# yardenas/ethz-safe-learning

Measured on AMD Instinct MI355X. Metric: planning steps/sec (CEM-MPC, N=2000 K=5 H=30), higher is better.
Workload: dtype f32

## Files before the change

### ethz_safe_learning_amd/_capi.py

```python
from __future__ import annotations

import ctypes as C
import os

CEM_ABI_VERSION = 4
CEM_MAX_ACT = 32
CEM_MAX_COST_KINDS = 4
CEM_COMM_ID_BYTES = 128
CEM_MAX_BATCH = 256
CEM_TRAIN_MAX_BATCH = 4096
CEM_INIT_COLD, CEM_INIT_EXPLICIT, CEM_INIT_SHIFT = 0, 1, 2
CEM_VARIANT_CEM, CEM_VARIANT_SAFE, CEM_VARIANT_COST = 0, 1, 2
CEM_PARTICLES_MEAN, CEM_PARTICLES_LOWER_TAIL = 0, 1
CEM_CONSTRAINT_BETA, CEM_CONSTRAINT_BUDGET = 0, 1
CEM_REFIT_UNIFORM, CEM_REFIT_SOFTMAX = 0, 1
CEM_NOISE_WHITE, CEM_NOISE_MIXED = 0, 1
CEM_FORWARD_SPLIT, CEM_FORWARD_ALL = 0, 1

_HERE = os.path.dirname(os.path.abspath(__file__))
LIB_PATH = os.environ.get('CEM_MPC_LIB') or os.path.join(_HERE, 'lib', 'libcem_mpc_gfx950.so')

EXPORTED_SYMBOLS = [
    'cem_abi_version', 'cem_status_string', 'cem_last_hip_error', 'cem_weight_blob_floats',
    'cem_packed_weight_floats', 'cem_workspace_bytes', 'cem_pack_weights_host', 'cem_plan_tiles_host', 'cem_plan_segments_host', 'cem_rollout_residency',
    'cem_planner_create', 'cem_planner_destroy', 'cem_planner_layout', 'cem_planner_set_weights', 'cem_planner_set_weights_dev',
    'cem_planner_set_normaliser', 'cem_planner_plan', 'cem_plan_begin', 'cem_plan_rollout', 'cem_plan_select',
    'cem_plan_end', 'cem_comm_unique_id', 'cem_planner_comm_init', 'cem_planner_comm_destroy', 'cem_planner_comm_ranks', 'cem_plan_exchange', 'cem_planner_graph_status', 'cem_planner_launches_per_iteration', 'cem_planner_rollout_path', 'cem_unfold_sequences', 'cem_compute_objective', 'cem_scorer_reward', 'cem_scorer_cost', 'cem_fill_noise', 'cem_philox_words', 'cem_planner_set_timing', 'cem_planner_last_timing', 'cem_planner_last_timing_detail', 'cem_planner_select_mode', 'cem_planner_inject_fault',
    'cem_batch_workspace_bytes', 'cem_batch_planner_create', 'cem_planner_plan_batch', 'cem_planner_batch_capacity',
    'cem_planner_set_warm_start', 'cem_planner_set_initial_distribution', 'cem_planner_set_init_mode', 'cem_planner_reset_carry',
    'cem_planner_get_carry', 'cem_planner_set_carry_slots', 'cem_planner_set_particle_objective', 'cem_planner_get_particle_objective',
    'cem_planner_set_constraint', 'cem_planner_get_constraint', 'cem_planner_set_cost_budget', 'cem_planner_constraint_costs',
    'cem_planner_set_refit', 'cem_planner_get_refit', 'cem_planner_refit_stats',
    'cem_planner_set_action_noise', 'cem_planner_get_action_noise', 'cem_planner_action_noise_dev',
    'cem_planner_set_elite_carry', 'cem_planner_get_elite_carry', 'cem_planner_elite_store',
    'cem_planner_set_population_schedule', 'cem_planner_get_population_schedule', 'cem_planner_iteration_plan',
    'cem_planner_set_mean_candidate', 'cem_planner_get_mean_candidate',
    'cem_trainer_workspace_bytes', 'cem_trainer_blob_floats', 'cem_trainer_create', 'cem_trainer_destroy', 'cem_trainer_set_state',
    'cem_trainer_get_state', 'cem_trainer_weights_dev', 'cem_trainer_step', 'cem_trainer_steps', 'cem_trainer_eval', 'cem_trainer_forward',
]


class CemScorer(C.Structure):
    _fields_ = [
        ('goal_mode', C.c_int32), ('goal_lo', C.c_int32), ('goal_hi', C.c_int32),
        ('lidar_max_dist', C.c_float), ('goal_size', C.c_float), ('goal_reached_dist', C.c_float), ('reward_distance', C.c_float),
        ('reward_goal', C.c_float), ('reward_clip', C.c_float),
        ('constrain_indicator', C.c_int32), ('n_cost_kinds', C.c_int32),
        ('cost_lo', C.c_int32 * CEM_MAX_COST_KINDS), ('cost_hi', C.c_int32 * CEM_MAX_COST_KINDS),
        ('cost_size', C.c_float * CEM_MAX_COST_KINDS),
    ]
# ... 74 lines not shown
    lib.cem_plan_tiles_host.argtypes = [cfgp, i32p, i32p, vp, C.c_int32]
    lib.cem_plan_segments_host.argtypes = [cfgp, i32p, i32p]
    lib.cem_rollout_residency.argtypes = [C.c_int32, C.c_int32, i32p, i32p]
    lib.cem_planner_create.argtypes = [cfgp, vp, C.c_size_t, vp, C.POINTER(vp)]
    lib.cem_planner_destroy.argtypes = [vp]
    lib.cem_planner_layout.argtypes = [vp, C.POINTER(CemLayout)]
    lib.cem_planner_set_weights.argtypes = [vp, vp, C.c_size_t]
    lib.cem_planner_set_weights_dev.argtypes = [vp, vp, C.c_size_t]
    lib.cem_planner_set_normaliser.argtypes = [vp, vp, vp]
    lib.cem_planner_plan.argtypes = [vp, vp, C.c_uint64, C.c_uint64, vp, vp, vp, vp, fp, i32p]
    lib.cem_plan_begin.argtypes = [vp, vp, C.c_uint64, C.c_uint64, vp, vp]
    lib.cem_plan_rollout.argtypes = [vp, C.c_int32]
    lib.cem_plan_select.argtypes = [vp, C.c_int32]
    lib.cem_plan_end.argtypes = [vp, vp, vp, fp, i32p]
    lib.cem_unfold_sequences.argtypes = [vp, vp, vp, C.c_int32, C.c_int32, vp, C.c_uint64, C.c_uint64, vp, vp, vp]
    lib.cem_comm_unique_id.argtypes = [vp]
    lib.cem_planner_comm_init.argtypes = [vp, vp, C.c_int32, C.c_int32]
    lib.cem_planner_comm_destroy.argtypes = [vp]
    lib.cem_plan_exchange.argtypes = [vp]
    lib.cem_planner_graph_status.argtypes = [vp, i32p]
    lib.cem_planner_comm_ranks.argtypes = [vp, i32p]
    lib.cem_planner_launches_per_iteration.argtypes = [vp, i32p]
    lib.cem_planner_rollout_path.argtypes = [vp, i32p]
    lib.cem_compute_objective.argtypes = [vp, vp, C.c_int32, C.c_int32, vp]
    lib.cem_scorer_reward.argtypes = [vp, vp, vp, C.c_int32, vp, vp]
    lib.cem_scorer_cost.argtypes = [vp, vp, C.c_int32, vp]
    lib.cem_fill_noise.argtypes = [vp, C.c_uint64, C.c_uint64, vp, vp, vp]
    lib.cem_philox_words.argtypes = [vp, C.c_uint64, C.c_uint64] + [C.c_uint32] * 6 + [vp]
    lib.cem_planner_select_mode.argtypes = [vp, i32p]
    lib.cem_planner_inject_fault.argtypes = [vp, C.c_int32]
    lib.cem_planner_set_timing.argtypes = [vp, C.c_int32]
    lib.cem_planner_last_timing.argtypes = [vp, fp, i32p, fp]
    lib.cem_planner_last_timing_detail.argtypes = [vp, fp, fp]
    lib.cem_batch_workspace_bytes.restype = C.c_size_t
    lib.cem_batch_workspace_bytes.argtypes = [cfgp, C.c_int32]
    lib.cem_batch_planner_create.argtypes = [cfgp, C.c_int32, vp, C.c_size_t, vp, C.POINTER(vp)]
    lib.cem_planner_plan_batch.argtypes = [vp, C.c_int32, vp, C.c_uint64, vp, vp, vp, vp, vp, vp, vp]
    lib.cem_planner_batch_capacity.argtypes = [vp, i32p]
    lib.cem_planner_set_warm_start.argtypes = [vp, C.POINTER(CemWarmStart)]
    lib.cem_planner_set_initial_distribution.argtypes = [vp, C.c_int32, vp, vp]
    lib.cem_planner_set_init_mode.argtypes = [vp, C.c_int32, C.c_int32]
    lib.cem_planner_reset_carry.argtypes = [vp, C.c_int32]
    lib.cem_planner_get_carry.argtypes = [vp, C.c_int32, vp, vp, i32p]
    lib.cem_planner_set_carry_slots.argtypes = [vp, C.c_int32, vp]
    lib.cem_planner_set_particle_objective.argtypes = [vp, C.c_int32, C.c_int32]
    lib.cem_planner_get_particle_objective.argtypes = [vp, i32p, i32p]
# ... 46 lines not shown
```

### ethz_safe_learning_amd/csrc/cem_capi.hip

```cpp
#include "cem_device.h"
#include "cem_rollout_lean.h"
#include "cem_score.h"
#include "cem_refit_weighted.h"
#include "cem_noise_mix.h"
#include "cem_elite_carry.h"
#include "cem_population.h"
#include "cem_train.h"
#include "cem_train_tile.h"
#include "cem_forward.h"
#include "cem_rollout_split.h"
#include "cem_rollout_wide.h"
#include "cem_pack.h"
#include "../../include/cem_mpc.h"

#include <dlfcn.h>
#include <link.h>

#include <algorithm>
#include <atomic>
#include <chrono>
#include <cmath>
#include <cstdio>
#include <cstdlib>
#include <cstring>
// ... 572 lines not shown
}

struct IterPlan {
    Dims d;
    int rc, n_tiles, n_seg, seg_len, n_pinned;
    bool sample_in_rollout, lean_rollout;
    size_t tiles_off;
};

struct cem_planner {
    cem_config_t cfg;
    Dims d;
    Layout lay;
    char *ws;
    hipStream_t stream;
    bool own_stream;
    int rc;
    int n_tiles;
    int n_seg, seg_len, n_pinned;
    bool have_weights;
    bool in_plan;
    bool sample_in_rollout;
    bool lean_rollout;
    const float *eps_act, *eps_model;
    CtrlBlock *h_ctrl;
    float *h_result;
    WarmCtl *h_warm; const WarmCtl *d_h_warm;
    uint32_t plan_seq;
    const CtrlBlock *d_h_ctrl; float *d_h_result;
    bool timing; std::vector<hipEvent_t> ev; float roll_ms, sel_ms, red_ms, samp_ms; int roll_n;
    std::vector<std::pair<int, int>> ev_kind;
    hipGraph_t graph; hipGraphExec_t gexec; bool graph_ready;
    ScorerDev sc;
    ScorerDev sc_roll;
    float alpha, beta;
    void *comm;
    int plans_since_comm;
    bool graph_failed;
    size_t sel_dyn_limit;
    int fused_resident;
    bool sel_zeroed;
    bool fuse_banned;
    bool inject_capture_fail;
    uint32_t inject_next;
    char *scratch; size_t scratch_bytes;
    std::vector<float> h_etab;
// ... 37 lines not shown

int warm_slots(const cem_planner *h) { return h->batch ? h->batch : 1; }

bool injects_mean(const cem_planner *h, int it) { return h->mean_cand && it == h->d.I - 1; }

struct IterView {
    const Dims *d; int rc, n_tiles, n_seg, seg_len, n_pinned; bool sample_in_rollout, lean_rollout;
    const TileDesc *tiles; uint32_t *seg_flags; f4 *seg_state;
};
IterView iter_view(const cem_planner *h, int it)
{
    const Layout &l = h->lay;
    if (h->pop.empty())
        return IterView{&h->d, h->rc, h->n_tiles, h->n_seg, h->seg_len, h->n_pinned, h->sample_in_rollout, h->lean_rollout,
                        (const TileDesc *)(h->ws + l.tiles), (uint32_t *)(h->ws + l.seg_flags), (f4 *)(h->ws + l.seg_state)};
    const IterPlan &ip = h->pop[std::min(std::max(it, 0), h->d.I - 1)];
    return IterView{&ip.d, ip.rc, ip.n_tiles, ip.n_seg, ip.seg_len, ip.n_pinned, ip.sample_in_rollout, ip.lean_rollout,
                    ip.tiles_off == (size_t)-1 ? (const TileDesc *)(h->ws + l.tiles) : (const TileDesc *)(h->pop_dev + ip.tiles_off),
                    h->pop_seg_flags, h->pop_seg_state};
}

bool samples_in_rollout(const cem_planner *h, int it) { return iter_view(h, it).sample_in_rollout && h->elite.n_keep == 0 && !injects_mean(h, it); }
bool runs_lean(const cem_planner *h, int it) { return iter_view(h, it).lean_rollout && h->elite.n_keep == 0 && !injects_mean(h, it); }
int32_t *elite_counts(const cem_planner *h) { return reinterpret_cast<int32_t *>(h->elite_dev); }
size_t elite_count_floats(const cem_planner *h) { return ((size_t)warm_slots(h) + 63) & ~(size_t)63; }
float *elite_store(const cem_planner *h) { return h->elite_dev + elite_count_floats(h); }

int select_mode_for(const cem_planner *h, int N, bool *cache = nullptr)
{
    const Dims &d = h->d;
    const bool can_fuse = (N + CEM_MS_KEYS - 1) / CEM_MS_KEYS <= h->fused_resident && !h->fuse_banned;
    return resolve_select_mode(h->cfg.select_mode, N, d.k, (long long)d.H * d.A, h->sel_dyn_limit, can_fuse, cache);
}
int select_mode_now(const cem_planner *h, bool *cache = nullptr) { return select_mode_for(h, h->d.N, cache); }

void drop_graph(cem_planner *h)
{
    if (h->gexec) { hipGraphExecDestroy(h->gexec); h->gexec = nullptr; }
    if (h->graph) { hipGraphDestroy(h->graph); h->graph = nullptr; }
    h->graph_ready = false;
}

int retire_graph(cem_planner *h)
{
    if (h->graph_ready) HIPCHK(hipStreamSynchronize(h->stream));
    drop_graph(h);
// ... 130 lines not shown
    if (const char *e = std::getenv("CEM_FORCE_ROLLOUT"))
        *lean_rollout = *lean_rollout && std::strcmp(e, "generic") != 0;
}

static int planner_create(const cem_config_t *cfg, int32_t mb, void *workspace, size_t workspace_bytes, void *hip_stream, cem_planner_t **out)
{
    int st = mb ? validate_batch(cfg, mb) : validate(cfg); if (st) return st;
    if (!workspace || !out) return CEM_ERR_INVALID_ARG;
    warn_if_two_hip_runtimes();
    cem_planner *h = new (std::nothrow) cem_planner();
    if (!h) return CEM_ERR_INVALID_ARG;
    h->cfg = *cfg; h->d = make_dims(cfg);
    h->batch = mb; h->n_states = warm_slots(h);
    const size_t nb = (size_t)warm_slots(h);
    h->lay = make_layout(cfg, h->d, max_tiles_of(h->d), mb);
    if (workspace_bytes < h->lay.total || ((uintptr_t)workspace & 255)) { delete h; return CEM_ERR_WORKSPACE; }
    h->ws = (char *)workspace; h->stream = (hipStream_t)hip_stream; h->own_stream = false;
    if (!h->stream) {
        if (hipStreamCreateWithFlags(&h->stream, hipStreamNonBlocking) != hipSuccess) { g_last_hip = (int)hipGetLastError(); delete h; return CEM_ERR_HIP; }
        h->own_stream = true;
    }
    { const Plan pl = make_plan(cfg, h->d, mb); h->rc = pl.rc; h->n_seg = pl.n_seg; h->seg_len = pl.seg_len; h->n_pinned = pl.n_pinned;
      place_sampler(h, h->d, pl, &h->sample_in_rollout, &h->lean_rollout); }
    h->have_weights = false; h->in_plan = false; h->eps_act = h->eps_model = nullptr;
    h->timing = false; h->roll_ms = h->sel_ms = h->red_ms = h->samp_ms = 0.f; h->roll_n = 0;
    h->graph = nullptr; h->gexec = nullptr; h->graph_ready = false; h->tail_m = 0;
    h->cost_m = 0; h->budget_dev = nullptr; h->cstat_obj = nullptr; h->cstat_obj_n = 0; h->last_cstat = nullptr; h->last_cstat_n = h->last_cstat_problems = 0;
    h->refit_kind = CEM_REFIT_UNIFORM; h->refit_tau = 0.f; h->refit_beta = 0.f; h->refit_dev = nullptr; h->refit_ran = false;
    h->noise_kind = CEM_NOISE_WHITE; h->noise_dev = nullptr; h->noise_eps = nullptr; h->noise_floats = 0;
    h->elite = cem_elite_carry_t{}; h->elite.shift = 1; h->elite_dev = nullptr; h->elite_cap = 0; h->elite_clear = false;
    h->pop_dev = nullptr; h->pop_seg_flags = nullptr; h->pop_seg_state = nullptr; h->pop_n_ready = 0; h->mean_cand = 0;
    h->h_budget.assign(nb, std::numeric_limits<float>::infinity());
    h->comm = nullptr; h->plans_since_comm = 0; h->graph_failed = false;
    h->h_ctrl = nullptr; h->h_result = nullptr; h->h_warm = nullptr; h->d_h_warm = nullptr; h->pack_desc = nullptr; h->n_pack_desc = 0;
    h->warm = cem_warm_start_t{}; h->warm.shift = 1; h->warm_staged = 0; h->warm_save_skipped = false;
    h->slot_mode.assign(nb, CEM_INIT_COLD); h->carry_valid.assign(nb, 0); h->have_expl.assign(nb, 0); h->carry_at.assign(nb, -1);
    h->slot_of.resize(nb); for (size_t b = 0; b < nb; ++b) h->slot_of[b] = (int32_t)b;
    h->h_expl.assign(nb * 2 * h->d.H * h->d.A, 0.f);
    h->scratch = nullptr; h->scratch_bytes = 0; h->sel_zeroed = false; h->plan_seq = 0; h->fuse_banned = false; h->inject_next = 0; h->inject_capture_fail = false;
    auto fail = [&](int status) { g_last_hip = (int)hipGetLastError(); release_handle(h); return status; };
    const size_t result_bytes = mb ? nb * CEM_RESULT_WORDS * 4 : 64 * 4;
    if (hipHostMalloc((void **)&h->h_ctrl, nb * sizeof(CtrlBlock), hipHostMallocMapped | hipHostMallocCoherent) != hipSuccess ||
        hipHostMalloc((void **)&h->h_result, result_bytes, hipHostMallocMapped | hipHostMallocCoherent) != hipSuccess ||
        hipHostMalloc((void **)&h->h_warm, sizeof(WarmCtl) + nb * sizeof(WarmProb), hipHostMallocMapped | hipHostMallocCoherent) != hipSuccess) return fail(CEM_ERR_HIP);
    {
        const std::vector<PackDesc> table = build_pack_table(h->d);
// ... 428 lines not shown
    if (!samples_in_rollout(h, it)) {
        const int total = d.N * d.H * ((d.A + 3) / 4);
        TimedLaunch timed(h, 3);
        hipLaunchKernelGGL(cem_sample_kernel, dim3(std::min((total + 255) / 256, 2048), nb), dim3(256), 0, h->stream, rp);
        HIPCHK(hipGetLastError());
        rp.musig = nullptr;
        if (h->elite.n_keep && (it > 0 || h->elite.across_plans)) {
            EliteCarryParams ep = fill_elite(h, it);
            HIPCHK(launch_elite_inject(ep, nb, h->stream));
        }
        if (injects_mean(h, it)) {
            MeanCandidateParams mc{}; mc.musig = (const float *)(ws + l.musig); mc.act_bounds = rp.act_bounds; mc.ctrl = rp.ctrl;
            mc.actions = rp.actions_w; mc.act_pad = rp.act_pad_w; mc.N = d.N; mc.row = d.N - 1; mc.H = d.H; mc.A = d.A;
            mc.pad_shift = rp.pad_shift; mc.pad_floats = rp.pad_floats;
            HIPCHK(launch_mean_candidate(mc, nb, h->stream));
        }
    }
    TimedLaunch timed(h, 0);
    if (runs_lean(h, it) && !rp.eps_act && !rp.eps_model) {
        if (queued) {
            rp.seg_queue = (uint32_t *)(ws + l.seg_queue); rp.seg_flags = v.seg_flags; rp.seg_state = v.seg_state;
            rp.seg_len = v.seg_len; rp.n_seg = v.n_seg; rp.n_pinned = v.n_pinned;
        }
        HIPCHK(launch_rollout_lean(rp, queued ? v.n_pinned + v.n_seg * (v.n_tiles - v.n_pinned) : v.n_tiles, h->stream, queued));
    }
    else if (d.wide) HIPCHK(launch_rollout_wide(h, rp, v.n_tiles, rp.eps_model ? 1 : 0));
    else if (d.split) HIPCHK(launch_rollout_split(v.rc, d.NFW, rp.eps_model ? 1 : 0, rp, v.n_tiles, h->stream));
    else if (rp.eps_model) HIPCHK(launch_rollout<1>(v.rc, d.NFW, rp, nb * v.n_tiles, h->stream));
    else if (queued) {
        rp.seg_queue = (uint32_t *)(ws + l.seg_queue); rp.seg_flags = v.seg_flags; rp.seg_state = v.seg_state;
        rp.seg_len = v.seg_len; rp.n_seg = v.n_seg; rp.n_pinned = v.n_pinned;
        HIPCHK(launch_rollout_seg(v.rc, d.NFW, rp, v.n_pinned + v.n_seg * (v.n_tiles - v.n_pinned), h->stream));
    } else HIPCHK(launch_rollout<0>(v.rc, d.NFW, rp, nb * v.n_tiles, h->stream));
    timed.stop();
    if (fold_reduce) return CEM_OK;

    const ReduceParams sp = fill_score(h, rp.ret, rp.costs, (float *)(ws + l.scores_local), h->cost_m ? h->budget_dev + nb : nullptr, d.Nloc, d.H, 1, true);
    h->sel_zeroed = true;
    if (h->cost_m) note_plan_cstat(h);
    TimedLaunch timed_reduce(h, 2);
    HIPCHK(launch_score(h, sp, nb));
    return CEM_OK;
}

bool folds_reduce(const cem_planner *h, int it = 0)
{
    const Dims &d = h->d;
// ... 881 lines not shown
    if (h->comm) {
        HIPCHK(hipStreamSynchronize(h->stream));
        if (Rccl *r = rccl()) r->CommDestroy(h->comm);
        h->comm = nullptr;
        drop_graph(h);
    }
    return CEM_OK;
}

int cem_planner_graph_status(const cem_planner_t *h, int32_t *status_out)
{
    if (!h || !status_out) return CEM_ERR_INVALID_ARG;
    *status_out = h->graph_ready ? 1 : (h->graph_failed ? 2 : 0);
    return CEM_OK;
}

int cem_planner_rollout_path(const cem_planner_t *h, int32_t *path_out)
{
    if (!h || !path_out) return CEM_ERR_INVALID_ARG;
    *path_out = (runs_lean(h, 0) && h->noise_kind != CEM_NOISE_MIXED) ? 1 : 0;
    return CEM_OK;
}

int cem_planner_launches_per_iteration(const cem_planner_t *h, int32_t *launches_out)
{
    if (!h || !launches_out) return CEM_ERR_INVALID_ARG;
    *launches_out = launches_of(h, 0);
    return CEM_OK;
}

int cem_planner_iteration_plan(const cem_planner_t *h, int32_t it, cem_iteration_plan_t *out)
{
    if (!h || !out || it < 0 || it >= h->d.I) return CEM_ERR_INVALID_ARG;
    const IterView v = iter_view(h, it);
    out->n_samples = v.d->N; out->chunks_per_tile = v.rc; out->n_tiles = v.n_tiles; out->n_segments = v.n_seg; out->n_pinned = v.n_pinned;
    out->launches = launches_of(h, it);
    out->rollout_path = (runs_lean(h, it) && h->noise_kind != CEM_NOISE_MIXED) ? 1 : 0;
    out->reserved = 0;
    return CEM_OK;
}

int cem_plan_exchange(cem_planner_t *h)
{
    if (!h) return CEM_ERR_INVALID_ARG;
    if (!h->in_plan || !h->comm) return CEM_ERR_STATE;
    return enqueue_exchange(h);
// ... 468 lines not shown
```

### ethz_safe_learning_amd/csrc/cem_rollout_lean.h

```cpp
#pragma once
#include "cem_device.h"

#define CEM_LEAN_ACT_LDS_BYTES(H_, AZ_) (((size_t)(H_) + 1) * (AZ_) * (32 + 17 * 16))
#define CEM_LEAN_LDS_BYTES(H_, AZ_) (CEM_ROLLOUT_LDS_BYTES(1) + CEM_LEAN_ACT_LDS_BYTES(H_, AZ_))
#define CEM_LEAN_ACT_LDS_MAX 16384

__attribute__((weak)) hipError_t launch_rollout_lean(const RolloutParams &p, int grid, hipStream_t st, bool seg);
```

### ethz_safe_learning_amd/planner.py

```python
from __future__ import annotations

import ctypes as C
import math
from dataclasses import dataclass, field
from typing import List, Optional, Sequence, Tuple

import numpy as np

from . import _capi


@dataclass
class ScorerConfig:
    goal_slice: Tuple[int, int]
    observe_goal_lidar: bool = True
    lidar_max_dist: float = 4.0
    goal_size: float = 0.3
    reward_distance: float = 1.0
    reward_goal: float = 1.0
    reward_clip: float = 10.0
    constrain_indicator: bool = True
    cost_kinds: List[Tuple[int, int, float]] = field(default_factory=list)


# ... 408 lines not shown
        n = C.c_int32()
        _capi.check(self.lib.cem_planner_comm_ranks(self.h, C.byref(n)), 'cem_planner_comm_ranks')
        return n.value

    def comm_destroy(self):
        _capi.check(self.lib.cem_planner_comm_destroy(self.h), 'cem_planner_comm_destroy')
        self.has_comm = False

    def graph_status(self):
        st = C.c_int32()
        _capi.check(self.lib.cem_planner_graph_status(self.h, C.byref(st)), 'cem_planner_graph_status')
        return ('eager', 'graph', 'graph-unsupported')[st.value]

    def launches_per_iteration(self):
        n = C.c_int32()
        _capi.check(self.lib.cem_planner_launches_per_iteration(self.h, C.byref(n)), 'cem_planner_launches_per_iteration')
        return n.value

    def rollout_path(self):
        n = C.c_int32()
        _capi.check(self.lib.cem_planner_rollout_path(self.h, C.byref(n)), 'cem_planner_rollout_path')
        return ('generic', 'lean')[n.value]

    def set_particle_objective(self, kind='mean', m=0):
        if kind not in PARTICLE_OBJECTIVES:
            raise ValueError("kind is 'mean' or 'lower_tail'")
        _capi.check(self.lib.cem_planner_set_particle_objective(self.h, PARTICLE_OBJECTIVES[kind], int(m)), 'cem_planner_set_particle_objective')

    def particle_objective(self):
        kind, m = C.c_int32(), C.c_int32()
        _capi.check(self.lib.cem_planner_get_particle_objective(self.h, C.byref(kind), C.byref(m)), 'cem_planner_get_particle_objective')
        return ('mean', 'lower_tail')[kind.value], m.value

    def set_constraint(self, kind='beta', worst_cost_particles=0):
        if kind not in CONSTRAINTS:
            raise ValueError("kind is 'beta' or 'budget'")
        _capi.check(self.lib.cem_planner_set_constraint(self.h, CONSTRAINTS[kind], int(worst_cost_particles)), 'cem_planner_set_constraint')

    def constraint(self):
        kind, m = C.c_int32(), C.c_int32()
        _capi.check(self.lib.cem_planner_get_constraint(self.h, C.byref(kind), C.byref(m)), 'cem_planner_get_constraint')
        return ('beta', 'budget')[kind.value], m.value

    def set_cost_budget(self, budget):
        b = np.ascontiguousarray(np.asarray(budget, np.float32).reshape(-1))
        self.budget_staged = None
# ... 567 lines not shown
```

### include/cem_mpc.h

```cpp
#ifndef CEM_MPC_H
#define CEM_MPC_H

#include <stddef.h>
#include <stdint.h>

#ifdef __cplusplus
extern "C" {
#endif

#define CEM_ABI_VERSION 4
#define CEM_MAX_ACT 32
#define CEM_MAX_COST_KINDS 4
#define CEM_MAX_BATCH 256

enum cem_status {
    CEM_OK = 0,
    CEM_ERR_INVALID_ARG = 1,
    CEM_ERR_UNSUPPORTED = 2,
    CEM_ERR_SPLIT = 3,
    CEM_ERR_WORKSPACE = 4,
    CEM_ERR_HIP = 5,
    CEM_ERR_NO_WEIGHTS = 6,
    CEM_ERR_STATE = 7,
    CEM_ERR_COMM = 8,
// ... 95 lines not shown
int cem_planner_set_weights_dev(cem_planner_t *h, const float *blob_dev, size_t n_floats);

int cem_planner_plan(cem_planner_t *h, const float *state, uint64_t seed, uint64_t call,
                     const float *eps_act_dev, const float *eps_model_dev, const float *eps_out_host,
                     float *action_out, float *best_score_out, int32_t *iters_out);

int cem_plan_begin(cem_planner_t *h, const float *state, uint64_t seed, uint64_t call,
                   const float *eps_act_dev, const float *eps_model_dev);
int cem_plan_rollout(cem_planner_t *h, int32_t it);
int cem_plan_select(cem_planner_t *h, int32_t it);
int cem_plan_end(cem_planner_t *h, const float *eps_out_host, float *action_out, float *best_score_out, int32_t *iters_out);

#define CEM_COMM_ID_BYTES 128
int cem_comm_unique_id(void *id_out );
int cem_planner_comm_init(cem_planner_t *h, const void *id , int32_t n_ranks, int32_t rank);
int cem_planner_comm_destroy(cem_planner_t *h);
int cem_planner_comm_ranks(const cem_planner_t *h, int32_t *n_ranks_out);
int cem_plan_exchange(cem_planner_t *h);
int cem_planner_select_mode(const cem_planner_t *h, int32_t *mode_out);
int cem_planner_inject_fault(cem_planner_t *h, int32_t kind);
int cem_planner_graph_status(const cem_planner_t *h, int32_t *status_out);
int cem_planner_launches_per_iteration(const cem_planner_t *h, int32_t *launches_out);
int cem_planner_rollout_path(const cem_planner_t *h, int32_t *path_out);

int cem_unfold_sequences(cem_planner_t *h, const float *s0_dev, const float *actions_dev, int32_t n_rows, int32_t horizon,
                         const float *eps_model_dev, uint64_t seed, uint64_t call,
                         float *traj_out_dev, float *mu_out_dev, float *sd_out_dev);

int cem_compute_objective(cem_planner_t *h, const float *traj_dev, int32_t n_rows, int32_t horizon, float *scores_out_dev);

int cem_scorer_reward(cem_planner_t *h, const float *obs_dev, const float *next_obs_dev, int32_t n, float *reward_out_dev,
                      uint8_t *goal_achieved_out_dev);
int cem_scorer_cost(cem_planner_t *h, const float *obs_dev, int32_t n, float *cost_out_dev);

int cem_fill_noise(cem_planner_t *h, uint64_t seed, uint64_t call, float *eps_act_dev, float *eps_model_dev, float *eps_out_dev);

int cem_philox_words(cem_planner_t *h, uint64_t seed, uint64_t call, uint32_t stream, uint32_t iteration, uint32_t t, uint32_t sub,
                     uint32_t idx0, uint32_t n, uint32_t *words_out_dev);

int cem_planner_set_timing(cem_planner_t *h, int32_t enable);
int cem_planner_last_timing(cem_planner_t *h, float *rollout_ms_total, int32_t *rollout_launches, float *select_ms_total);
int cem_planner_last_timing_detail(cem_planner_t *h, float *reduce_ms_total, float *sampler_ms_total);

size_t cem_batch_workspace_bytes(const cem_config_t *cfg, int32_t max_batch);
int cem_batch_planner_create(const cem_config_t *cfg, int32_t max_batch, void *workspace, size_t workspace_bytes, void *hip_stream,
                             cem_planner_t **out);
// ... 96 lines not shown
```

Measured before the change: 542.2.

## Add straight-line specialized lean rollout kernel with ring-buffered weight prefetch

Adds a specialized lean rollout kernel for the common configuration (4 layers, one forward wave, no goal mode, at most one cost). It fully unrolls the MLP stages at compile time and streams weight groups through a four-slot register ring of buffer loads issued several groups ahead, so the generic kernel's runtime branching and load latency stall less on the matrix cores. The dispatcher selects it when the configuration matches, with an environment override to force the old branchy path. It adds a large amount of duplicated kernel code and some risk of register pressure or correctness drift from the generic path.

```diff
diff --git a/ethz_safe_learning_amd/_capi.py b/ethz_safe_learning_amd/_capi.py
--- a/ethz_safe_learning_amd/_capi.py
+++ b/ethz_safe_learning_amd/_capi.py
@@ -25,7 +25,7 @@
     'cem_packed_weight_floats', 'cem_workspace_bytes', 'cem_pack_weights_host', 'cem_plan_tiles_host', 'cem_plan_segments_host', 'cem_rollout_residency',
     'cem_planner_create', 'cem_planner_destroy', 'cem_planner_layout', 'cem_planner_set_weights', 'cem_planner_set_weights_dev',
     'cem_planner_set_normaliser', 'cem_planner_plan', 'cem_plan_begin', 'cem_plan_rollout', 'cem_plan_select',
-    'cem_plan_end', 'cem_comm_unique_id', 'cem_planner_comm_init', 'cem_planner_comm_destroy', 'cem_planner_comm_ranks', 'cem_plan_exchange', 'cem_planner_graph_status', 'cem_planner_launches_per_iteration', 'cem_planner_rollout_path', 'cem_unfold_sequences', 'cem_compute_objective', 'cem_scorer_reward', 'cem_scorer_cost', 'cem_fill_noise', 'cem_philox_words', 'cem_planner_set_timing', 'cem_planner_last_timing', 'cem_planner_last_timing_detail', 'cem_planner_select_mode', 'cem_planner_inject_fault',
+    'cem_plan_end', 'cem_comm_unique_id', 'cem_planner_comm_init', 'cem_planner_comm_destroy', 'cem_planner_comm_ranks', 'cem_plan_exchange', 'cem_planner_graph_status', 'cem_planner_launches_per_iteration', 'cem_planner_rollout_path', 'cem_planner_rollout_form', 'cem_unfold_sequences', 'cem_compute_objective', 'cem_scorer_reward', 'cem_scorer_cost', 'cem_fill_noise', 'cem_philox_words', 'cem_planner_set_timing', 'cem_planner_last_timing', 'cem_planner_last_timing_detail', 'cem_planner_select_mode', 'cem_planner_inject_fault',
     'cem_batch_workspace_bytes', 'cem_batch_planner_create', 'cem_planner_plan_batch', 'cem_planner_batch_capacity',
     'cem_planner_set_warm_start', 'cem_planner_set_initial_distribution', 'cem_planner_set_init_mode', 'cem_planner_reset_carry',
     'cem_planner_get_carry', 'cem_planner_set_carry_slots', 'cem_planner_set_particle_objective', 'cem_planner_get_particle_objective',
@@ -146,6 +146,7 @@
     lib.cem_planner_comm_ranks.argtypes = [vp, i32p]
     lib.cem_planner_launches_per_iteration.argtypes = [vp, i32p]
     lib.cem_planner_rollout_path.argtypes = [vp, i32p]
+    lib.cem_planner_rollout_form.argtypes = [vp, C.c_int32, i32p]
     lib.cem_compute_objective.argtypes = [vp, vp, C.c_int32, C.c_int32, vp]
     lib.cem_scorer_reward.argtypes = [vp, vp, vp, C.c_int32, vp, vp]
     lib.cem_scorer_cost.argtypes = [vp, vp, C.c_int32, vp]
diff --git a/ethz_safe_learning_amd/csrc/cem_capi.hip b/ethz_safe_learning_amd/csrc/cem_capi.hip
--- a/ethz_safe_learning_amd/csrc/cem_capi.hip
+++ b/ethz_safe_learning_amd/csrc/cem_capi.hip
@@ -618,6 +618,7 @@
     bool in_plan;
     bool sample_in_rollout;
     bool lean_rollout;
+    bool lean_branchy;
     const float *eps_act, *eps_model;
     CtrlBlock *h_ctrl;
     float *h_result;
@@ -701,6 +702,14 @@
 
 bool samples_in_rollout(const cem_planner *h, int it) { return iter_view(h, it).sample_in_rollout && h->elite.n_keep == 0 && !injects_mean(h, it); }
 bool runs_lean(const cem_planner *h, int it) { return iter_view(h, it).lean_rollout && h->elite.n_keep == 0 && !injects_mean(h, it); }
+
+int lean_form(const cem_planner *h, int it)
+{
+    const Dims &d = *iter_view(h, it).d; const ScorerDev &sc = h->sc_roll;
+    bool straight = launch_rollout_lean_straight != nullptr && !h->lean_branchy && !sc.goal_mode && sc.n_cost <= 1 && d.L == 4 && d.NFW == 1;
+    for (int w = 0; w < 4; ++w) straight = straight && d.wave_groups[w] == 4 + 3 * CEM_NG + (w < d.KB_obs ? CEM_NG : 0);
+    return straight ? 2 : 1;
+}
 int32_t *elite_counts(const cem_planner *h) { return reinterpret_cast<int32_t *>(h->elite_dev); }
 size_t elite_count_floats(const cem_planner *h) { return ((size_t)warm_slots(h) + 63) & ~(size_t)63; }
 float *elite_store(const cem_planner *h) { return h->elite_dev + elite_count_floats(h); }
@@ -877,6 +886,7 @@
     }
     { const Plan pl = make_plan(cfg, h->d, mb); h->rc = pl.rc; h->n_seg = pl.n_seg; h->seg_len = pl.seg_len; h->n_pinned = pl.n_pinned;
       place_sampler(h, h->d, pl, &h->sample_in_rollout, &h->lean_rollout); }
+    { const char *e = std::getenv("CEM_FORCE_ROLLOUT"); h->lean_branchy = e && std::strcmp(e, "lean_branchy") == 0; }
     h->have_weights = false; h->in_plan = false; h->eps_act = h->eps_model = nullptr;
     h->timing = false; h->roll_ms = h->sel_ms = h->red_ms = h->samp_ms = 0.f; h->roll_n = 0;
     h->graph = nullptr; h->gexec = nullptr; h->graph_ready = false; h->tail_m = 0;
@@ -1351,7 +1361,9 @@
             rp.seg_queue = (uint32_t *)(ws + l.seg_queue); rp.seg_flags = v.seg_flags; rp.seg_state = v.seg_state;
             rp.seg_len = v.seg_len; rp.n_seg = v.n_seg; rp.n_pinned = v.n_pinned;
         }
-        HIPCHK(launch_rollout_lean(rp, queued ? v.n_pinned + v.n_seg * (v.n_tiles - v.n_pinned) : v.n_tiles, h->stream, queued));
+        const int grid = queued ? v.n_pinned + v.n_seg * (v.n_tiles - v.n_pinned) : v.n_tiles;
+        if (lean_form(h, it) == 2 && (rp.variant == 1) == (rp.costs != nullptr)) HIPCHK(launch_rollout_lean_straight(rp, grid, h->stream, queued));
+        else HIPCHK(launch_rollout_lean(rp, grid, h->stream, queued));
     }
     else if (d.wide) HIPCHK(launch_rollout_wide(h, rp, v.n_tiles, rp.eps_model ? 1 : 0));
     else if (d.split) HIPCHK(launch_rollout_split(v.rc, d.NFW, rp.eps_model ? 1 : 0, rp, v.n_tiles, h->stream));
@@ -2279,6 +2291,13 @@
     return CEM_OK;
 }
 
+int cem_planner_rollout_form(const cem_planner_t *h, int32_t it, int32_t *form_out)
+{
+    if (!h || !form_out || it < 0 || it >= h->d.I) return CEM_ERR_INVALID_ARG;
+    *form_out = (runs_lean(h, it) && h->noise_kind != CEM_NOISE_MIXED) ? lean_form(h, it) : 0;
+    return CEM_OK;
+}
+
 int cem_planner_launches_per_iteration(const cem_planner_t *h, int32_t *launches_out)
 {
     if (!h || !launches_out) return CEM_ERR_INVALID_ARG;
diff --git a/ethz_safe_learning_amd/csrc/cem_rollout_lean.h b/ethz_safe_learning_amd/csrc/cem_rollout_lean.h
--- a/ethz_safe_learning_amd/csrc/cem_rollout_lean.h
+++ b/ethz_safe_learning_amd/csrc/cem_rollout_lean.h
@@ -6,3 +6,4 @@
 #define CEM_LEAN_ACT_LDS_MAX 16384
 
 __attribute__((weak)) hipError_t launch_rollout_lean(const RolloutParams &p, int grid, hipStream_t st, bool seg);
+__attribute__((weak)) hipError_t launch_rollout_lean_straight(const RolloutParams &p, int grid, hipStream_t st, bool seg);
diff --git a/ethz_safe_learning_amd/csrc/cem_rollout_lean_straight.hip b/ethz_safe_learning_amd/csrc/cem_rollout_lean_straight.hip
--- /dev/null
+++ b/ethz_safe_learning_amd/csrc/cem_rollout_lean_straight.hip
@@ -0,0 +1,412 @@
+#define CEM_DEVICE_PRIMITIVES_ONLY
+#include "cem_rollout_lean.h"
+
+namespace {
+
+template <int V> struct StraightConst { static constexpr int value = V; };
+
+constexpr int SL_GROUPS_BODY = 4 + 3 * CEM_NG, SL_GROUPS_HEADS = SL_GROUPS_BODY + CEM_NG;
+
+struct StraightRing {
+    __amdgpu_buffer_rsrc_t rsrc;
+    int voff, n;
+    AGroup slot[4];
+    template <int G> __device__ __forceinline__ AGroup ld() const
+    {
+        const int g = G < SL_GROUPS_BODY ? G : (G >= n ? G - n : G);
+        const int soff = (g >> 1) * 4096;
+        constexpr int half = (G & 1) * 2048;
+        AGroup r;
+        r.a = __builtin_bit_cast(f4, __builtin_amdgcn_raw_buffer_load_b128(rsrc, voff + half, soff, 0));
+        r.b = __builtin_bit_cast(f4, __builtin_amdgcn_raw_buffer_load_b128(rsrc, voff + half + 1024, soff, 0));
+        return r;
+    }
+    __device__ __forceinline__ void init(const f4 *b, int lane_, int n_)
+    {
+        rsrc = __builtin_amdgcn_make_buffer_rsrc(const_cast<f4 *>(b), 0, n_ * 2048, 0x00020000);
+        voff = lane_ * 16; n = n_;
+        slot[0] = ld<0>(); slot[1] = ld<1>(); slot[2] = ld<2>(); slot[3] = slot[2];
+    }
+};
+
+template <int KF, int NOWN, bool L0IN, int BASE>
+__device__ __forceinline__ void cem_straight_stage(f4 (&acc0)[1], f4 (&acc1)[1], f4 (&hB)[CEM_NG][1], StraightRing &wq, const char *const *rb, const int xoff)
+{
+    static_assert(KF % 4 == 0 && BASE % 4 == 0, "stage lengths must keep the ring phase");
+    auto group = [&](auto PC) __attribute__((always_inline)) {
+        constexpr int P = decltype(PC)::value;
+        wq.slot[(P + 3) & 3] = wq.template ld<BASE + P + 3>();
+        __builtin_amdgcn_sched_barrier(0);
+        if (P == 1) {
+            __syncthreads();
+#pragma unroll
+            for (int Q = NOWN; Q < KF; ++Q) hB[Q][0] = *reinterpret_cast<const f4 *>(rb[Q - NOWN] + xoff + (Q - NOWN) * 1024);
+        }
+        const AGroup g = wq.slot[P & 3];
+        constexpr int Pb = (!L0IN && P < 2) ? (P ^ 1) : P;
+#pragma unroll
+        for (int r = 0; r < 4; ++r) {
+            acc0[0] = CEM_MFMA(g.a[r], hB[P][0][r], acc0[0]);
+            acc1[0] = CEM_MFMA(g.b[r], hB[Pb][0][r], acc1[0]);
+        }
+    };
+    group(StraightConst<0>{}); group(StraightConst<1>{}); group(StraightConst<2>{}); group(StraightConst<3>{});
+    if constexpr (KF == 8) { group(StraightConst<4>{}); group(StraightConst<5>{}); group(StraightConst<6>{}); group(StraightConst<7>{}); }
+}
+
+template <bool SEG, bool SAFE>
+__device__ __forceinline__ void cem_straight_tile(const RolloutParams &p, char *smem, const int tile_idx, const int t_begin, const int t_end)
+{
+    constexpr int RC = 1;
+    const int tid = (int)((threadIdx.x + 64u * (unsigned)((tile_idx + (tile_idx >> 8)) & 3)) & 255u);
+    const int w = __builtin_amdgcn_readfirstlane(tid >> 6);
+    const int lane = tid & 63;
+    const int j = lane & 15, q = lane >> 4;
+    const TileDesc td = p.tiles[tile_idx];
+    const bool resumed = SEG && t_begin > 0;
+    const bool bkwave = w == 0;
+    auto seg_buffer = [&]() __attribute__((always_inline)) {
+        return __builtin_amdgcn_make_buffer_rsrc(
+            SEG ? const_cast<f4 *>(p.seg_state + (size_t)(tile_idx - p.n_pinned) * (2 * 256 + 64)) : const_cast<f4 *>(p.wpack), 0, (2 * 256 + 64) * 16, 0x00020000);
+    };
+    const int O = p.O, A = p.A, H = p.H, AZ = (A + 3) >> 2;
+    constexpr int XB = CEM_NG * 1024;
+    float *part = reinterpret_cast<float *>(smem + 2 * XB);
+    const CtrlBlock *const ctrl = p.ctrl;
+    const PhiloxKey key = cem_key(ctrl);
+    const float rscale = p.sampling ? CEM_BM_RSCALE : 0.0f;
+
+    const int member_u = __builtin_amdgcn_readfirstlane(td.member);
+    const bool heads = w < p.KB_obs;
+    StraightRing wq;
+    wq.init(p.wpack + (size_t)member_u * p.member_stride_f4 + p.wave_off_f4[w], lane, heads ? SL_GROUPS_HEADS : SL_GROUPS_BODY);
+
+    const __amdgpu_buffer_rsrc_t et_rs = __builtin_amdgcn_make_buffer_rsrc(
+        const_cast<float *>(p.etab + (size_t)member_u * (CEM_ET_ROWS + p.L) * CEM_U), 0, (CEM_ET_ROWS + p.L) * CEM_U * 4, 0x00020000);
+    const int tab_v = 64 * w + 16 * q;
+    const int bias_v = 128 * w + 16 * q;
+    const char *tabl = smem + 2 * XB + CEM_PART_FLOATS * 4;
+    const char *actl = tabl + CEM_TAB_LDS_BYTES;
+    {
+        const int ht = (int)threadIdx.x;
+        *reinterpret_cast<f4 *>(const_cast<char *>(tabl) + ht * 16) = cem_ld_tab(et_rs, (ht & 31) * 16, (ht >> 5) * 512);
+        const int HA = H * A;
+        for (int idx = ht; idx < (H + 1) * AZ; idx += 256) {
+            const int t = idx / AZ, z = idx - t * AZ;
+            const float *lo = t < H ? p.musig + HA + t * A : p.act_bounds, *hi = t < H ? p.musig + t * A : p.act_bounds + 32;
+            f4 u = {0.f, 0.f, 0.f, 0.f}, v = u;
+#pragma unroll
+            for (int r = 0; r < 4; ++r) if (4 * z + r < A) { u[r] = lo[4 * z + r]; v[r] = hi[4 * z + r]; }
+            *reinterpret_cast<f4 *>(const_cast<char *>(actl) + idx * 32) = u;
+            *reinterpret_cast<f4 *>(const_cast<char *>(actl) + idx * 32 + 16) = v;
+        }
+    }
+    __syncthreads();
+
+    f4 s;
+    const int slot0 = j < td.cnt ? j : td.cnt - 1;
+    {
+        const int f0 = 16 * w + 4 * q;
+        if (resumed) s = cem_ld_coherent(seg_buffer(), tid * 16);
+        else {
+#pragma unroll
+            for (int r = 0; r < 4; ++r) {
+                const int f = f0 + r;
+                float v = 0.f;
+                if (f < O) v = td.s0_base < 0 ? ctrl->state[f] : p.s0[(size_t)(td.s0_base + slot0) * O + f];
+                s[r] = v;
+            }
+        }
+    }
+
+    const int zq = 4 * w + q - (O >> 2);
+    const bool actlane = zq >= 0 && zq < AZ;
+    const bool wact = 4 * w + 3 >= (O >> 2) && 4 * w < (O >> 2) + AZ;
+    const int zc = actlane ? zq : 0;
+    const uint32_t pc0 = (uint32_t)((actlane ? td.act_base : td.noise_row_base) + slot0);
+    const uint32_t pc2 = actlane ? ((uint32_t)zc | (CEM_STREAM_ACT << 16)) : ((uint32_t)(4 * w + q) | (CEM_STREAM_MODEL << 16));
+    const uint32_t pc1 = ((uint32_t)p.it << 16) + (actlane ? 1u : 0u);
+    const float prs = actlane ? CEM_BM_RSCALE : rscale;
+    const char *const actl_v = actl + zc * 32;
+#define CEM_LEAN_ACTION(DST, E_, T_) do { \
+        const char *m_ = actl_v + (T_) * AZ * 32, *b_ = actl_v + H * AZ * 32; \
+        const f4 sg_ = *reinterpret_cast<const f4 *>(m_), mu_ = *reinterpret_cast<const f4 *>(m_ + 16); \
+        const f4 lb_ = *reinterpret_cast<const f4 *>(b_), ub_ = *reinterpret_cast<const f4 *>(b_ + 16); \
+        f4 v_ = (E_) * sg_; v_ = v_ + mu_; \
+        _Pragma("unroll") for (int r = 0; r < 4; ++r) DST[r] = fminf(fmaxf(v_[r], lb_[r]), ub_[r]); } while (0)
+    const bool act_keep = actlane && j < td.cnt && td.row_base < p.Nloc;
+    char *const stage = const_cast<char *>(actl) + (H + 1) * AZ * 32;
+    char *const stage_v = stage + ((act_keep ? j : 16) * (H + 1) * AZ + zc) * 16;
+#define CEM_LEAN_KEEP(V_, T_) do { *reinterpret_cast<f4 *>(stage_v + (T_) * AZ * 16) = (V_); } while (0)
+
+    const float scD = p.sc.D, goal_thresh = p.sc.goal_thresh, reward_distance = p.sc.reward_distance, reward_goal = p.sc.reward_goal;
+    const float clipv = p.sc.reward_clip > 0.f ? p.sc.reward_clip : __builtin_inff();
+    const float csz0 = p.sc.n_cost > 0 ? p.sc.cost_size[0] : -__builtin_inff();
+    float d_prev = 0.f, c_prev = 0.f, cum = 0.f;
+    bool done = false;
+
+    auto terms = [&](float &dn, float &cn) __attribute__((always_inline)) {
+        dn = CEM_PART_MIN4(part, lane, 0);
+        const float dk = CEM_PART_MIN4(part, lane, 1);
+        cn = (dk <= csz0) ? 1.0f : 0.0f;
+    };
+    auto settle = [&](const float dn, const float cn, const int T) __attribute__((always_inline)) {
+        const bool ga = d_prev <= goal_thresh;
+        float r = (d_prev - dn) * reward_distance + (ga ? 1.0f : 0.0f) * reward_goal;
+        r = fminf(fmaxf(r, -clipv), clipv);
+        if (SAFE) {
+            done = done || ga;
+            const float nd = done ? 0.0f : 1.0f;
+            const float cst = c_prev * nd;
+            if (lane < td.cnt) {
+                const __amdgpu_buffer_rsrc_t cost_rs = __builtin_amdgcn_make_buffer_rsrc(p.costs, 0, (uint32_t)(H * p.Bloc), 0x00020000);
+                __builtin_amdgcn_raw_buffer_store_b8((uint8_t)cst, cost_rs, td.row_base + lane, __builtin_amdgcn_readfirstlane(T * p.Bloc), 0);
+            }
+            cum = cum + r * nd;
+        } else {
+            const float nd = done ? 0.0f : 1.0f;
+            cum = cum + r * nd;
+            done = done || ga;
+        }
+        d_prev = dn; c_prev = cn;
+    };
+
+    f4 hB[CEM_NG][RC];
+    if (resumed) {
+        const __amdgpu_buffer_rsrc_t seg_rs = seg_buffer();
+        const f4 x = cem_ld_coherent(seg_rs, (256 + tid) * 16);
+        hB[0][0] = x;
+        *reinterpret_cast<f4 *>(smem + (w * 64 + lane) * 16) = x;
+        if (bkwave) {
+            const f4 b = cem_ld_coherent(seg_rs, (2 * 256 + lane) * 16);
+            d_prev = b[0]; c_prev = b[1]; cum = b[2]; done = b[3] != 0.f;
+        }
+    } else {
+        float pm0 = __builtin_inff(), pm1 = __builtin_inff();
+        const int tv = tab_v;
+        const f4 mn4 = CEM_TAB(tabl, CEM_ET_NMIN, tv), rd4 = CEM_TAB(tabl, CEM_ET_RDELTA, tv);
+        const f4 isact4 = CEM_TAB(tabl, CEM_ET_ACT, tv);
+        const f4 sel0 = CEM_TAB(tabl, CEM_ET_SEL0, tv), sel1 = CEM_TAB(tabl, CEM_ET_SEL1, tv);
+        const f4 e0 = cem_normal4(pc0, 0u, (uint32_t)p.it, (uint32_t)zc, CEM_STREAM_ACT, key);
+        const f4 sn = s;
+        f4 xin = sn;
+        if (wact) {
+            f4 act4; CEM_LEAN_ACTION(act4, e0, 0);
+            CEM_LEAN_KEEP(act4, 0);
+            xin = __builtin_elementwise_fma(isact4, act4, sn);
+        }
+        cem_scorer_terms(sn, scD, sel0, sel1, pm0, pm1);
+        const f4 x = cem_sub4(xin, mn4) * rd4;
+        *reinterpret_cast<f4 *>(smem + (w * 64 + lane) * 16) = x;
+        hB[0][0] = x;
+        CEM_PAIR_MIN_STORE(part, w, q, j, 0, pm0, pm1, true, 0);
+    }
+    f4 nb0 = cem_ld_tab(et_rs, bias_v, CEM_ET_ROWS * 512);
+    f4 nb1 = cem_ld_tab(et_rs, bias_v + 64, CEM_ET_ROWS * 512);
+
+    const char *rbh[6], *rb0[3];
+#pragma unroll
+    for (int k = 0; k < 6; ++k) rbh[k] = smem + lane * 16 + (k < 2 * w ? 0 : 2048);
+#pragma unroll
+    for (int k = 0; k < 3; ++k) rb0[k] = smem + lane * 16 + (k < w ? 0 : 1024);
+    char *const pubh = smem + (2 * w * 64 + lane) * 16, *const pub0 = smem + (w * 64 + lane) * 16;
+    static_assert(CEM_FLOAT_PRIO == 3, "level 3 of the step's priority switch is the floating segments' priority");
+    int lvl = (SEG && tile_idx >= p.n_pinned) ? 3 : (t_begin + (tile_idx >> 8) % 3) % 3;
+    auto step = [&](auto XW0, const int t, const bool first) __attribute__((always_inline)) {
+        int xw = decltype(XW0)::value;
+        if (lvl < 2) { if (lvl == 0) __builtin_amdgcn_s_setprio(0); else __builtin_amdgcn_s_setprio(1); }
+        else { if (lvl == 2) __builtin_amdgcn_s_setprio(2); else __builtin_amdgcn_s_setprio(3); }
+        lvl = lvl == 2 ? 0 : (lvl == 3 ? 3 : lvl + 1);
+        asm volatile("" : "+s"(lvl));
+#define CEM_RELU_PUBLISH() do { \
+            f4 h0 = acc0[0], h1 = acc1[0]; \
+            _Pragma("unroll") for (int r = 0; r < 4; ++r) { h0[r] = fmaxf(h0[r], 0.f); h1[r] = fmaxf(h1[r], 0.f); } \
+            *reinterpret_cast<f4 *>(pubh + xw) = h0; \
+            *reinterpret_cast<f4 *>(pubh + xw + 1024) = h1; \
+            hB[0][0] = h0; hB[1][0] = h1; \
+            xw ^= XB; } while (0)
+#define CEM_NEXT_BIAS(LN) do { \
+            nb0 = cem_ld_tab(et_rs, bias_v, (CEM_ET_ROWS + (LN)) * 512); \
+            nb1 = cem_ld_tab(et_rs, bias_v + 64, (CEM_ET_ROWS + (LN)) * 512); } while (0)
+        {
+            f4 acc0[RC], acc1[RC];
+            acc0[0] = nb0; acc1[0] = nb1;
+            CEM_NEXT_BIAS(1);
+            cem_straight_stage<4, 1, true, 0>(acc0, acc1, hB, wq, rb0, xw ^ XB);
+            if (bkwave) {
+                if (first) {
+                    if (!resumed) terms(d_prev, c_prev);
+                } else {
+                    float dn, cn;
+                    terms(dn, cn);
+                    settle(dn, cn, t - 1);
+                }
+            }
+            CEM_RELU_PUBLISH();
+        }
+        {
+            f4 acc0[RC], acc1[RC];
+            acc0[0] = nb0; acc1[0] = nb1;
+            CEM_NEXT_BIAS(2);
+            cem_straight_stage<CEM_NG, 2, false, 4>(acc0, acc1, hB, wq, rbh, xw ^ XB);
+            CEM_RELU_PUBLISH();
+        }
+        {
+            f4 acc0[RC], acc1[RC];
+            acc0[0] = nb0; acc1[0] = nb1;
+            CEM_NEXT_BIAS(3);
+            cem_straight_stage<CEM_NG, 2, false, 12>(acc0, acc1, hB, wq, rbh, xw ^ XB);
+            CEM_RELU_PUBLISH();
+        }
+        {
+            f4 acc0[RC], acc1[RC];
+            acc0[0] = nb0; acc1[0] = nb1;
+            CEM_NEXT_BIAS(0);
+            cem_straight_stage<CEM_NG, 2, false, 20>(acc0, acc1, hB, wq, rbh, xw ^ XB);
+            CEM_RELU_PUBLISH();
+        }
+#undef CEM_RELU_PUBLISH
+#undef CEM_NEXT_BIAS
+
+        float pm0 = __builtin_inff(), pm1 = __builtin_inff();
+        const int tn = (t + 1 < H) ? t + 1 : H - 1;
+        {
+            const int tv = tab_v;
+            f4 accm[RC], accv[RC];
+            accm[0] = CEM_TAB(tabl, CEM_ET_BMU, tv); accv[0] = CEM_TAB(tabl, CEM_ET_BVAR, tv);
+            if (heads) cem_straight_stage<CEM_NG, 2, false, 28>(accm, accv, hB, wq, rbh, xw ^ XB);
+            else __syncthreads();
+            const f4 e4 = cem_normal4(pc0, pc1 + (uint32_t)t, 0u, pc2, 0u, key, prs);
+            const f4 mn4 = CEM_TAB(tabl, CEM_ET_NMIN, tv), rd4 = CEM_TAB(tabl, CEM_ET_RDELTA, tv);
+            const f4 om4 = CEM_TAB(tabl, CEM_ET_OBS, tv);
+            const f4 sel0 = CEM_TAB(tabl, CEM_ET_SEL0, tv), sel1 = CEM_TAB(tabl, CEM_ET_SEL1, tv);
+
+            const f4 mu = accm[0];
+            const f4 var = cem_softplus4(accv[0]) + 1e-4f;
+            f4 sd;
+#pragma unroll
+            for (int r = 0; r < 4; ++r) sd[r] = __builtin_amdgcn_sqrtf(var[r]);
+            const f4 d = mu + sd * e4;
+            const f4 sn = s + d * om4;
+            s = sn;
+            cem_scorer_terms(sn, scD, sel0, sel1, pm0, pm1);
+            if (wact) {
+                const f4 isact4 = CEM_TAB(tabl, CEM_ET_ACT, tv);
+                f4 act4; CEM_LEAN_ACTION(act4, e4, tn);
+                CEM_LEAN_KEEP(act4, t + 1);
+                const f4 x = cem_sub4(__builtin_elementwise_fma(isact4, act4, sn), mn4) * rd4;
+                *reinterpret_cast<f4 *>(pub0 + xw) = x;
+                hB[0][0] = x;
+            } else {
+                const f4 x = cem_sub4(sn, mn4) * rd4;
+                *reinterpret_cast<f4 *>(pub0 + xw) = x;
+                hB[0][0] = x;
+            }
+        }
+        CEM_PAIR_MIN_STORE(part, w, q, j, 0, pm0, pm1, true, 0);
+    };
+    for (int t = t_begin; t < t_end; t += 2) {
+        step(StraightConst<XB>{}, t, t == t_begin);
+        if (t + 1 >= t_end) break;
+        step(StraightConst<0>{}, t + 1, false);
+    }
+#undef CEM_LEAN_ACTION
+#undef CEM_LEAN_KEEP
+    __syncthreads();
+    if (bkwave) {
+        float dn, cn;
+        terms(dn, cn);
+        settle(dn, cn, t_end - 1);
+    }
+    if (td.row_base < p.Nloc) {
+        const int tlo = resumed ? t_begin + 1 : 0, thi = t_end < H ? t_end : H - 1;
+        const int per = (thi - tlo + 1) * A;
+        const float *const stagef = reinterpret_cast<const float *>(stage);
+        for (int idx = (int)threadIdx.x; idx < td.cnt * per; idx += 256) {
+            const int row = idx / per, rem = idx - row * per, tt = tlo + rem / A, a = rem - (rem / A) * A;
+            p.actions_w[((size_t)(td.act_base + row) * H + tt) * A + a] = stagef[((row * (H + 1) + tt) * AZ) * 4 + a];
+        }
+    }
+    if (!SEG || t_end == H) {
+        if (bkwave && lane < td.cnt) p.ret[td.row_base + lane] = cum;
+    } else {
+        const __amdgpu_buffer_rsrc_t seg_rs = seg_buffer();
+        cem_st_coherent(seg_rs, tid * 16, s);
+        cem_st_coherent(seg_rs, (256 + tid) * 16, hB[0][0]);
+        if (bkwave) cem_st_coherent(seg_rs, (2 * 256 + lane) * 16, (f4){d_prev, c_prev, cum, done ? 1.0f : 0.0f});
+    }
+}
+
+}
+
+template <bool SAFE>
+__global__ __launch_bounds__(256) void cem_rollout_lean_straight_kernel(const RolloutParams p)
+{
+    extern __shared__ __attribute__((aligned(16))) char smem[];
+    if (p.check_done && p.ctrl->done) return;
+    cem_straight_tile<false, SAFE>(p, smem, (int)blockIdx.x, 0, p.H);
+}
+
+template <bool SAFE>
+__global__ __launch_bounds__(256) void cem_rollout_lean_straight_seg_kernel(const RolloutParams p)
+{
+    extern __shared__ __attribute__((aligned(16))) char smem[];
+    __shared__ uint32_t item_s;
+    if (p.check_done && p.ctrl->done) return;
+    if ((int)blockIdx.x < p.n_pinned) {
+        cem_straight_tile<true, SAFE>(p, smem, (int)blockIdx.x, 0, p.H);
+        return;
+    }
+    __builtin_amdgcn_s_setprio(CEM_FLOAT_PRIO);
+    const uint32_t n_float = (uint32_t)(p.n_tiles - p.n_pinned);
+    if (threadIdx.x == 0) {
+        const uint32_t ticket = atomicAdd(p.seg_queue, 1u);
+        uint32_t item = (((uint32_t)p.n_pinned + ticket) << 8);
+        if (ticket >= n_float) {
+            const uint32_t *slot = p.seg_flags + (ticket - n_float);
+            uint32_t spins = 0, v;
+            while ((v = __hip_atomic_load(slot, __ATOMIC_RELAXED, __HIP_MEMORY_SCOPE_AGENT)) == 0u && ++spins < CEM_SEG_SPIN_LIMIT)
+                __builtin_amdgcn_s_sleep(16);
+            item = v ? v - 1u : 0xffffffffu;
+            if (!v) atomicOr(const_cast<int32_t *>(&p.ctrl->fault), 1 );
+        }
+        item_s = item;
+    }
+    __syncthreads();
+    const uint32_t item = item_s;
+    if (item == 0xffffffffu) return;
+    const int tile = (int)(item >> 8), seg = (int)(item & 255u);
+    const int t0 = seg * p.seg_len, t1 = (t0 + p.seg_len < p.H) ? t0 + p.seg_len : p.H;
+    cem_straight_tile<true, SAFE>(p, smem, tile, t0, t1);
+    if (t1 == p.H) {
+        if (threadIdx.x == 0) item_s = atomicAdd(p.seg_queue + 2, 1u);
+        __syncthreads();
+        if (item_s == n_float - 1u) {
+            const int n_ready = (int)n_float * (p.n_seg - 1);
+            for (int i = (int)threadIdx.x; i < n_ready; i += 256) __hip_atomic_store(p.seg_flags + i, 0u, __ATOMIC_RELAXED, __HIP_MEMORY_SCOPE_AGENT);
+            if (threadIdx.x < 3) __hip_atomic_store(p.seg_queue + threadIdx.x, 0u, __ATOMIC_RELAXED, __HIP_MEMORY_SCOPE_AGENT);
+        }
+    }
+    if (t1 < p.H) {
+        __builtin_amdgcn_s_waitcnt(0x0F70);
+        __syncthreads();
+        if (threadIdx.x == 0) {
+            const uint32_t pos = atomicAdd(p.seg_queue + 1, 1u);
+            __hip_atomic_store(p.seg_flags + pos, (((uint32_t)tile << 8) | (uint32_t)(seg + 1)) + 1u, __ATOMIC_RELAXED, __HIP_MEMORY_SCOPE_AGENT);
+        }
+    }
+}
+
+hipError_t launch_rollout_lean_straight(const RolloutParams &p, int grid, hipStream_t st, bool seg)
+{
+    const size_t lds = CEM_LEAN_LDS_BYTES(p.H, (p.A + 3) / 4);
+    const bool safe = p.variant == 1;
+    if (seg) {
+        if (safe) hipLaunchKernelGGL(cem_rollout_lean_straight_seg_kernel<true>, dim3(grid), dim3(256), lds, st, p);
+        else hipLaunchKernelGGL(cem_rollout_lean_straight_seg_kernel<false>, dim3(grid), dim3(256), lds, st, p);
+    } else {
+        if (safe) hipLaunchKernelGGL(cem_rollout_lean_straight_kernel<true>, dim3(grid), dim3(256), lds, st, p);
+        else hipLaunchKernelGGL(cem_rollout_lean_straight_kernel<false>, dim3(grid), dim3(256), lds, st, p);
+    }
+    return hipGetLastError();
+}
diff --git a/ethz_safe_learning_amd/planner.py b/ethz_safe_learning_amd/planner.py
--- a/ethz_safe_learning_amd/planner.py
+++ b/ethz_safe_learning_amd/planner.py
@@ -454,6 +454,11 @@
         _capi.check(self.lib.cem_planner_rollout_path(self.h, C.byref(n)), 'cem_planner_rollout_path')
         return ('generic', 'lean')[n.value]
 
+    def rollout_form(self, it=0):
+        n = C.c_int32()
+        _capi.check(self.lib.cem_planner_rollout_form(self.h, int(it), C.byref(n)), 'cem_planner_rollout_form')
+        return n.value
+
     def set_particle_objective(self, kind='mean', m=0):
         if kind not in PARTICLE_OBJECTIVES:
             raise ValueError("kind is 'mean' or 'lower_tail'")
diff --git a/include/cem_mpc.h b/include/cem_mpc.h
--- a/include/cem_mpc.h
+++ b/include/cem_mpc.h
@@ -141,6 +141,7 @@
 int cem_planner_graph_status(const cem_planner_t *h, int32_t *status_out);
 int cem_planner_launches_per_iteration(const cem_planner_t *h, int32_t *launches_out);
 int cem_planner_rollout_path(const cem_planner_t *h, int32_t *path_out);
+int cem_planner_rollout_form(const cem_planner_t *h, int32_t it, int32_t *form_out);
 
 int cem_unfold_sequences(cem_planner_t *h, const float *s0_dev, const float *actions_dev, int32_t n_rows, int32_t horizon,
                          const float *eps_model_dev, uint64_t seed, uint64_t call,
```

After: 551.8 (median of 6 runs). +1.8%, better.
